# chriskery/slurm-bridge-operator

Measured on AMD Instinct MI355X. Metric: placements/sec + job×node fit evals/sec, 100k nodes×1M jobs, 1–8 MI355X, higher is better.
Workload: dtype int32

## Files before the change

### slurm-bridge-operator_amd/csrc/engine.cpp

```cpp
#include <errno.h>
#include <fcntl.h>
#include <hip/hip_runtime_api.h>
#include <hip/hip_vector_types.h>
#include <rccl/rccl.h>
#include <sys/file.h>
#include <sys/stat.h>
#include <unistd.h>

#include <algorithm>
#include <chrono>
#include <cstdarg>
#include <cstdio>
#include <cstdlib>
#include <cstring>
#include <initializer_list>
#include <map>
#include <mutex>
#include <new>
#include <string>
#include <vector>

#include "../../include/fitgpu.h"
#include "fit_device.h"

using namespace fitgpu;

namespace {

inline int64_t ring_comps(int nc) {
    const int g = std::max(1, std::min(engine_ring_groups(), nc));
    return (nc + g - 1) / g;
}

thread_local std::string g_last_error;

int fail(int code, const char* fmt, ...) {
    char buf[512];
    va_list ap;
    va_start(ap, fmt);
    vsnprintf(buf, sizeof buf, fmt, ap);
    va_end(ap);
    g_last_error = buf;
    return code;
}

#define HIP_TRY(expr)                                                                       \
    do {                                                                                    \
        hipError_t e_ = (expr);                                                             \
        if (e_ != hipSuccess)                                                               \
            return fail(FIT_E_HIP, "%s failed: %s (%s:%d)", #expr, hipGetErrorString(e_),   \
                        __FILE__, __LINE__);                                                \
    } while (0)

#define NCCL_TRY(expr)                                                                      \
    do {                                                                                    \
        ncclResult_t r_ = (expr);                                                           \
        if (r_ != ncclSuccess)                                                              \
            return fail(FIT_E_RCCL, "%s failed: %s", #expr, ncclGetErrorString(r_));        \
    } while (0)

template <class T>
struct DBuf {
    T* p = nullptr;
    size_t cap = 0;
    int ensure(size_t n) {
        if (n <= cap) return 0;
        if (p) (void)hipFree(p);
        p = nullptr;
        cap = 0;
        size_t want = std::max<size_t>(n, 64);
        if (hipMalloc(&p, want * sizeof(T)) != hipSuccess) {
            p = nullptr;
            return fail(FIT_E_OOM, "hipMalloc(%zu bytes) failed", want * sizeof(T));
        }
        cap = want;
        return 0;
    }
    void release() {
        if (p) (void)hipFree(p);
        p = nullptr;
        cap = 0;
    }
    DBuf() = default;
    DBuf(const DBuf&) = delete;
    DBuf& operator=(const DBuf&) = delete;
    ~DBuf() { release(); }
};

template <class T>
struct HBuf {
    T* p = nullptr;
    size_t cap = 0;
    int ensure(size_t n) {
        if (n <= cap) return 0;
        if (p) (void)hipHostFree(p);
        p = nullptr;
        cap = 0;
        size_t want = std::max<size_t>(n, 64);
        if (hipHostMalloc(&p, want * sizeof(T), hipHostMallocDefault) != hipSuccess) {
            p = nullptr;
            return fail(FIT_E_OOM, "hipHostMalloc(%zu bytes) failed", want * sizeof(T));
        }
        cap = want;
        return 0;
    }
    void release() {
        if (p) (void)hipHostFree(p);
        p = nullptr;
        cap = 0;
    }
    HBuf() = default;
    HBuf(const HBuf&) = delete;
    HBuf& operator=(const HBuf&) = delete;
    ~HBuf() { release(); }
};

template <class Row>
struct QueryBufs {
    DBuf<Row> out;
    DBuf<int32_t> bad;
    HBuf<Row> h;
    double ms = -1;
};

int find_root(int* par, int x) {
    while (par[x] != x) x = par[x] = par[par[x]];
    return x;
}

double now_ms() {
    using namespace std::chrono;
    return duration<double, std::milli>(steady_clock::now().time_since_epoch()).count();
}

struct DevArb {
    std::mutex mu;
    int fd = -1;
    std::string path;
};

constexpr const char* FIT_LOCK_DIR_DEFAULT = "/var/run/fitgpu";
int resolve_lock_dir(std::string& dir) {
    const char* e = getenv("FIT_LOCK_DIR");
    if (e && *e) {
        dir = e;
        return 0;
    }
    struct stat sb;
    if (stat(FIT_LOCK_DIR_DEFAULT, &sb) == 0 && S_ISDIR(sb.st_mode)) {
        dir = FIT_LOCK_DIR_DEFAULT;
        return 0;
    }
    dir = "/tmp";
    return 1;
}

DevArb* dev_arb(int device, std::string& err) {
    static std::mutex m;
    static std::map<int, DevArb*> tab;
    std::lock_guard<std::mutex> g(m);
    DevArb*& a = tab[device];
    if (!a) a = new DevArb();
    if (a->fd < 0) {
        char bus[64] = {0};
        if (hipDeviceGetPCIBusId(bus, sizeof bus, device) != hipSuccess) snprintf(bus, sizeof bus, "dev%d", device);
        for (char* q = bus; *q; ++q)
            if (*q == ':' || *q == '/') *q = '_';
        std::string dir;
        (void)resolve_lock_dir(dir);
        a->path = dir + "/fitgpu-" + bus + ".lock";
        a->fd = open(a->path.c_str(), O_RDWR | O_CREAT | O_CLOEXEC, 0666);
        if (a->fd >= 0) (void)fchmod(a->fd, 0666);
        else a->fd = open(a->path.c_str(), O_RDONLY | O_CLOEXEC);
        if (a->fd < 0) {
            err = a->path + ": " + strerror(errno);
            return nullptr;
        }
    }
    return a;
}

struct ArbGuard {
    DevArb* a = nullptr;
    double waited_ms = 0;
    int take(int device) {
        const double t0 = now_ms();
        std::string err;
        DevArb* d = dev_arb(device, err);
        if (!d) return fail(FIT_E_STATE, "device lock %s (set FIT_LOCK_DIR to a writable directory)", err.c_str());
        d->mu.lock();
        int r;
        do r = flock(d->fd, LOCK_EX);
        while (r != 0 && errno == EINTR);
        if (r != 0) {
            d->mu.unlock();
            return fail(FIT_E_STATE, "flock %s: %s", d->path.c_str(), strerror(errno));
        }
        a = d;
        waited_ms = now_ms() - t0;
        return 0;
    }
    ~ArbGuard() {
        if (!a) return;
        (void)flock(a->fd, LOCK_UN);
        a->mu.unlock();
    }
};

}

struct CtxHandles {
    ncclComm_t comm = nullptr;
    hipStream_t st = nullptr;
    hipEvent_t ev[6] = {};
    hipStream_t st2 = nullptr;
    hipEvent_t ev_join = nullptr;
    unsigned* resident = nullptr;
    CtxHandles() = default;
    CtxHandles(const CtxHandles&) = delete;
    CtxHandles& operator=(const CtxHandles&) = delete;
    ~CtxHandles() {
        for (auto& e : ev)
            if (e) (void)hipEventDestroy(e);
        if (ev_join) (void)hipEventDestroy(ev_join);
        if (resident) (void)hipHostFree(resident);
        if (st2) (void)hipStreamDestroy(st2);
        if (st) (void)hipStreamDestroy(st);
        if (comm) (void)ncclCommDestroy(comm);
    }
};

struct fit_ctx : CtxHandles {
    int device = 0;
    int rank = 0, world = 1;
    int shard_mode = FIT_SHARD_AUTO;
    fit_exchange_fn xchg = nullptr;
    void* xchg_user = nullptr;
    HBuf<uint8_t> h_x;
    DBuf<uint64_t> xcount;
    bool force_coll = false;
    bool collective() const { return world > 1 || force_coll; }
    bool persistent = true;
    int32_t small_batch = 2048;
    int32_t small_direct = 128;
    bool small_args = true, sync_spin = true;
    int cls_mode = 3;
    int32_t last_multi = 0;
    bool cls_nodes_ok = false;
    int32_t cls_maxn = 0;
    DBuf<int16_t> jcls;
    DBuf<uint8_t> cls_tab;
    DBuf<int4> cls_dem;
    DBuf<int32_t> cls_n;
    DBuf<unsigned> cls_err;
    HBuf<int32_t> h_cls_n;
    HBuf<unsigned> h_cls_err;
    DBuf<int32_t> small_placed;
    HBuf<int32_t> h_small;
    DBuf<uint8_t> jpack;
    HBuf<uint8_t> h_jpack;
    QueryBufs<fit_why> ex;
    QueryBufs<fit_eta> wh;
    QueryBufs<struct fit_room> rm;
    QueryBufs<fit_eta_k> wk;
    DBuf<int32_t> wk_node, wk_diff;
    HBuf<int32_t> h_wk_node;
    DBuf<unsigned long long> wk_top;
    DBuf<int32_t> ptlk_cnt;
    HBuf<int32_t> h_ptlk;
    DBuf<int32_t> tlr_node, tlr_start, tlr_state, tlr_inv, tlr_cnt, tlr_first, tlr_fill, tlr_touched, tlr_flag, tlr_g;
    DBuf<TlWin> tlr_win;
    DBuf<unsigned long long> tlr_tot;
    HBuf<int32_t> h_tlr_g;
    HBuf<unsigned long long> h_tlr_tot;
    double utl_ms = -1, htl_ms = -1;
    DBuf<int32_t> atl_tc, atl_tm, atl_tg, atl_g;
    HBuf<int32_t> h_atl;
    double atl_ms = -1;
    DBuf<int64_t> free_acc;
    DBuf<fit_free> free_rows;
    double free_ms = -1;
    DBuf<int32_t> vs_off, vs_prio, vs_cpu, vs_mem, vs_gpu, vic_bad, voff;
    HBuf<int32_t> h_vic_bad;
    DBuf<VicEnt> vent;
    bool have_vic = false;
    QueryBufs<fit_evict> pe;
    DBuf<int32_t> pe_prio;
    HBuf<int32_t> h_pe_prio;
    DBuf<uint4> pe_part;
    QueryBufs<fit_evict_k> pk;
    DBuf<int32_t> pk_node, pk_vic;
    HBuf<int32_t> h_pk_pick;
    int cus = 256;
    DBuf<uint8_t> ectl, ering;
    DBuf<CompState> ecs;
    DBuf<CompOut> eco;
    DBuf<int64_t> ebusy;
    HBuf<CompState> h_ecs;
    HBuf<CompOut> h_eco;
    HBuf<int64_t> h_ebusy;
    HBuf<uint32_t> h_err;
    HBuf<TripRec> h_trip;
    DBuf<NodeRec> rec_bak;
    unsigned wd_ticks = 1000000000u;
    HBuf<uint64_t> h_count;
    int wmin = 256, wmax = 8192;

    int32_t n = 0;
    int32_t nn = 0;
    int ncomp = 0;
    int comp_of_part[32];
    std::vector<int32_t> nb;
    DBuf<NodeRec> rec;
    DBuf<int32_t> col_cpu, col_mem, col_gpu, col_av, perm;
    DBuf<uint32_t> col_mask;
    DBuf<int32_t> rb_cpu, rb_mem, rb_gpu;
    std::vector<uint32_t> h_mask;
    std::vector<int32_t> h_perm;
    bool have_nodes = false;
    int64_t loads = 0;

    int32_t np = 0;
    int32_t ptab[128];
    DBuf<int32_t> d_ptab;

    DBuf<int32_t> jcpu, jmem, jgpu, jwall, out, jl, jpk;
    DBuf<uint16_t> jpart, jk;
    DBuf<int8_t> jcomp;
    DBuf<int32_t> jmin;
    DBuf<uint64_t> cand, bnd;
    DBuf<JobRec> wjob;
    DBuf<CompPlan> plan;
    DBuf<CommitResult> res;
    HBuf<CompPlan> h_plan;
    HBuf<CommitResult> h_res;
    DBuf<int32_t> jls;
    HBuf<int32_t> h_jls;

    int32_t tl_slots = 0, tl_slot_min = 0;
    bool have_tl = false;
    DBuf<Seg> slab;
    DBuf<TlHdr> tlhdr;
    DBuf<int32_t> outs, rel_off, rel_slot, rel_cpu, rel_mem, rel_gpu;
    DBuf<uint32_t> tl_err;
    HBuf<uint32_t> h_tl_err;
};

namespace {

int build_ptab(fit_ctx* c) {
    for (int p = 0; p < 32; ++p) c->ptab[96 + p] = c->comp_of_part[p];
    if (c->d_ptab.ensure(128)) return FIT_E_OOM;
    HIP_TRY(hipMemcpyAsync(c->d_ptab.p, c->ptab, sizeof c->ptab, hipMemcpyHostToDevice, c->st));
    return 0;
}

int load_nodes_common(fit_ctx* c, int32_t n) {
    int par[32];
    for (int i = 0; i < 32; ++i) par[i] = i;
    bool used[32] = {false};
    for (int32_t x = 0; x < n; ++x) {
        uint32_t m = c->h_mask[x];
        if (!m) continue;
        int lo = __builtin_ctz(m);
        for (uint32_t r = m; r; r &= r - 1) {
            int b = __builtin_ctz(r);
            used[b] = true;
            int ra = find_root(par, lo), rb = find_root(par, b);
            if (ra != rb) par[std::max(ra, rb)] = std::min(ra, rb);
        }
    }
    int root_comp[32];
    for (int i = 0; i < 32; ++i) root_comp[i] = -1;
    c->ncomp = 0;
    for (int p = 0; p < 32; ++p) {
        c->comp_of_part[p] = -1;
        if (!used[p]) continue;
        int r = find_root(par, p);
        if (root_comp[r] < 0) root_comp[r] = c->ncomp++;
        c->comp_of_part[p] = root_comp[r];
    }
    c->nb.assign(c->ncomp + 1, 0);
    for (int32_t x = 0; x < n; ++x)
        if (c->h_mask[x]) c->nb[c->comp_of_part[__builtin_ctz(c->h_mask[x])] + 1]++;
    for (int k = 0; k < c->ncomp; ++k) {
        if (c->nb[k + 1] > MAX_COMPONENT_NODES)
            return fail(FIT_E_INVAL, "partition component %d has %d nodes (limit %d)", k,
                        c->nb[k + 1], MAX_COMPONENT_NODES);
        c->nb[k + 1] += c->nb[k];
    }
    c->nn = c->nb[c->ncomp];
    {
        int parts_of[32] = {0};
        for (int p = 0; p < 32; ++p)
            if (c->comp_of_part[p] >= 0) ++parts_of[c->comp_of_part[p]];
        c->cls_nodes_ok = c->ncomp > 0 && c->ncomp <= 32;
        c->cls_maxn = 0;
        for (int k = 0; k < c->ncomp; ++k) {
            const int32_t nk = c->nb[k + 1] - c->nb[k];
            c->cls_maxn = std::max(c->cls_maxn, nk);
            if (parts_of[k] != 1) c->cls_nodes_ok = false;
        }
        if (c->cls_maxn > class_max_nodes() || class_lds_bytes(c->cls_maxn) > 160 * 1024)
            c->cls_nodes_ok = false;
    }
    std::vector<int32_t> fill(c->nb.begin(), c->nb.end() - 1), perm(std::max(c->nn, 1));
    for (int32_t x = 0; x < n; ++x)
        if (c->h_mask[x]) perm[fill[c->comp_of_part[__builtin_ctz(c->h_mask[x])]]++] = x;
    if (c->perm.ensure(std::max(c->nn, 1)) || c->rec.ensure(std::max(c->nn, 1))) return FIT_E_OOM;
    HIP_TRY(hipMemcpyAsync(c->perm.p, perm.data(), sizeof(int32_t) * c->nn, hipMemcpyHostToDevice,
                           c->st));
    HIP_TRY(launch_gather_nodes(c->st, c->col_cpu.p, c->col_mem.p, c->col_gpu.p, c->col_av.p,
                                c->col_mask.p, c->perm.p, c->nn, c->rec.p));
    int rc = build_ptab(c);
    if (rc) return rc;
    HIP_TRY(hipStreamSynchronize(c->st));
    perm.resize(c->nn);
    c->h_perm.swap(perm);
    c->n = n;
    c->have_nodes = true;
    c->have_tl = false;
    ++c->loads;
    return 0;
}

int alloc_cols(fit_ctx* c, int32_t n) {
    size_t m = std::max<int32_t>(n, 1);
    if (c->col_cpu.ensure(m) || c->col_mem.ensure(m) || c->col_gpu.ensure(m) ||
        c->col_av.ensure(m) || c->col_mask.ensure(m))
        return FIT_E_OOM;
    return 0;
}

int xchg(fit_ctx* c, int op, void* dbuf, int64_t count) {
    if (!c->collective() || count == 0) return 0;
    if (!c->xchg) {
        switch (op) {
            case FIT_XCHG_ALLGATHER_U64: {
                uint64_t* b = static_cast<uint64_t*>(dbuf);
                NCCL_TRY(ncclAllGather(b + (size_t)c->rank * count, b, count, ncclUint64, c->comm,
                                       c->st));
                return 0;
            }
            case FIT_XCHG_MIN_U64:
                NCCL_TRY(ncclAllReduce(dbuf, dbuf, count, ncclUint64, ncclMin, c->comm, c->st));
                return 0;
            case FIT_XCHG_MAX_I32:
                NCCL_TRY(ncclAllReduce(dbuf, dbuf, count, ncclInt32, ncclMax, c->comm, c->st));
                return 0;
            case FIT_XCHG_MIN_I32:
                NCCL_TRY(ncclAllReduce(dbuf, dbuf, count, ncclInt32, ncclMin, c->comm, c->st));
                return 0;
        }
        return fail(FIT_E_INVAL, "exchange op %d", op);
    }
    const size_t elem = (op == FIT_XCHG_ALLGATHER_U64 || op == FIT_XCHG_MIN_U64) ? 8 : 4;
    const size_t bytes = elem * (size_t)count * (op == FIT_XCHG_ALLGATHER_U64 ? c->world : 1);
    if (c->h_x.ensure(bytes)) return FIT_E_OOM;
    HIP_TRY(hipMemcpyAsync(c->h_x.p, dbuf, bytes, hipMemcpyDeviceToHost, c->st));
    HIP_TRY(hipStreamSynchronize(c->st));
    if (c->xchg(c->xchg_user, op, c->h_x.p, count) != 0)
        return fail(FIT_E_RCCL, "host exchange op %d failed", op);
    HIP_TRY(hipMemcpyAsync(dbuf, c->h_x.p, bytes, hipMemcpyHostToDevice, c->st));
    return 0;
}

const char* trip_site_name(unsigned s) {
    switch (s) {
        case TRIP_WORKER_RING: return "scan worker waiting for a task";
        case TRIP_ROUND_START: return "committer waiting for the round before last";
        case TRIP_HELPER_TILE: return "commit helper waiting for a scan tile";
        case TRIP_HELPER_SNAP: return "commit helper waiting for the decider";
        case TRIP_DECIDER_REC: return "decider waiting for a helper record";
        case TRIP_SINGLE_TILE: return "single-wave commit waiting for a scan tile";
        case TRIP_NO_PROGRESS: return "round resolved no job";
// ... 1326 lines not shown
        c->comp_of_part[p] = -1;
        c->ptab[p] = c->ptab[32 + p] = c->ptab[64 + p] = -1;
        c->ptab[96 + p] = -1;
    }
    int rc = 0;
    if (hipStreamCreateWithFlags(&c->st, hipStreamNonBlocking) != hipSuccess) rc = FIT_E_HIP;
    for (auto& e : c->ev)
        if (!rc && hipEventCreate(&e) != hipSuccess) rc = FIT_E_HIP;
    if (!rc && c->world == 1 && c->force_coll && !c->xchg) {
        ncclUniqueId id;
        ncclResult_t r = ncclGetUniqueId(&id);
        if (r == ncclSuccess) r = ncclCommInitRank(&c->comm, 1, id, 0);
        if (r != ncclSuccess) rc = fail(FIT_E_RCCL, "ncclCommInitRank(1 rank): %s", ncclGetErrorString(r));
    } else if (!rc && c->world > 1 && !c->xchg) {
        if (!o.nccl_id) {
            rc = fail(FIT_E_INVAL, "world > 1 needs nccl_id");
        } else {
            ncclUniqueId id;
            memcpy(&id, o.nccl_id, sizeof id);
            ncclResult_t r = ncclCommInitRank(&c->comm, c->world, id, c->rank);
            if (r != ncclSuccess)
                rc = fail(FIT_E_RCCL, "ncclCommInitRank: %s", ncclGetErrorString(r));
        }
    } else if (rc) {
        fail(rc, "stream/event creation failed");
    }
    if (rc) {
        delete c;
        return rc;
    }
    *out_ctx = c;
    return 0;
}

int fit_set_watchdog_us(fit_ctx* c, int64_t us) {
    if (!c) return fail(FIT_E_INVAL, "null ctx");
    if (us <= 0) {
        c->wd_ticks = 1000000000u;
        if (const char* ev = getenv("FIT_WATCHDOG_MS"))
            c->wd_ticks = (unsigned)std::min<double>(4.29e9, std::max(1.0, atof(ev) * 1e5));
        return 0;
    }
    c->wd_ticks = (unsigned)std::min<int64_t>(us * 100, 4290000000ll);
    return 0;
}

void fit_destroy(fit_ctx* ctx) {
    if (!ctx) return;
    (void)hipSetDevice(ctx->device);
    (void)hipStreamSynchronize(ctx->st);
    delete ctx;
}

static int load_node_cols(fit_ctx* c, int32_t n, const int32_t* cpu, const int32_t* mem, const int32_t* gpu,
                          const int32_t* av, const uint32_t* mask, hipMemcpyKind kind) {
    if (!c) return fail(FIT_E_INVAL, "null ctx");
    if (n < 0 || n > FIT_MAX_NODES || (n > 0 && (!cpu || !mem || !gpu || !av || !mask)))
        return fail(FIT_E_INVAL, "bad node arrays");
    c->have_nodes = c->have_tl = false;
    c->have_vic = false;
    HIP_TRY(hipSetDevice(c->device));
    if (alloc_cols(c, n)) return FIT_E_OOM;
    const size_t b = sizeof(int32_t) * n;
    HIP_TRY(hipMemcpyAsync(c->col_cpu.p, cpu, b, kind, c->st));
    HIP_TRY(hipMemcpyAsync(c->col_mem.p, mem, b, kind, c->st));
    HIP_TRY(hipMemcpyAsync(c->col_gpu.p, gpu, b, kind, c->st));
    HIP_TRY(hipMemcpyAsync(c->col_av.p, av, b, kind, c->st));
    HIP_TRY(hipMemcpyAsync(c->col_mask.p, mask, b, kind, c->st));
    return 0;
}

int fit_load_nodes(fit_ctx* c, int32_t n, const int32_t* cpu, const int32_t* mem,
                   const int32_t* gpu, const int32_t* av, const uint32_t* mask) {
    const int rc = load_node_cols(c, n, cpu, mem, gpu, av, mask, hipMemcpyHostToDevice);
    if (rc) return rc;
    c->h_mask.assign(mask, mask + n);
    return load_nodes_common(c, n);
}

int fit_load_nodes_device(fit_ctx* c, int32_t n, const int32_t* cpu, const int32_t* mem,
                          const int32_t* gpu, const int32_t* av, const uint32_t* mask) {
    const int rc = load_node_cols(c, n, cpu, mem, gpu, av, mask, hipMemcpyDeviceToDevice);
    if (rc) return rc;
    c->h_mask.resize(n);
    HIP_TRY(hipMemcpyAsync(c->h_mask.data(), mask, sizeof(uint32_t) * n, hipMemcpyDeviceToHost, c->st));
    HIP_TRY(hipStreamSynchronize(c->st));
    return load_nodes_common(c, n);
}

int fit_load_partitions(fit_ctx* c, int32_t p, const int32_t* max_time,
                        const int32_t* max_cpus, const int32_t* max_mem) {
    if (!c) return fail(FIT_E_INVAL, "null ctx");
    if (p < 0 || p > FIT_MAX_PARTITIONS || (p > 0 && (!max_time || !max_cpus || !max_mem)))
        return fail(FIT_E_INVAL, "bad partition table (p=%d)", p);
    HIP_TRY(hipSetDevice(c->device));
    c->np = p;
    for (int i = 0; i < 32; ++i) {
        c->ptab[i] = i < p ? max_time[i] : -1;
        c->ptab[32 + i] = i < p ? max_cpus[i] : -1;
        c->ptab[64 + i] = i < p ? max_mem[i] : -1;
    }
    int rc = build_ptab(c);
    if (rc) return rc;
    HIP_TRY(hipStreamSynchronize(c->st));
    return 0;
}

static int check_place_args(fit_ctx* c, int32_t j, std::initializer_list<const void*> arrays, int32_t kmax) {
    const int rc = check_job_args(c, j, arrays, nullptr, 0);
    if (rc) return rc;
    if (kmax < 1 || kmax > FIT_MAX_K)
        return fail(FIT_E_INVAL, "kmax=%d outside [1, %d]", kmax, FIT_MAX_K);
    return 0;
}

constexpr int32_t kPackJobs = 16384;

int fit_place(fit_ctx* c, int32_t j, const int32_t* cpu, const int32_t* mem, const int32_t* gpu,
              const int32_t* wall, const uint16_t* part, const uint16_t* nk, int32_t kmax,
              int32_t* out, fit_stats* stats) {
    int rc = check_place_args(c, j, {cpu, mem, gpu, wall, part, out}, kmax);
    if (rc) return rc;
    HIP_TRY(hipSetDevice(c->device));
    size_t m = std::max(j, 1);
    if (c->out.ensure(m * kmax + 2 + FIT_MAX_PARTITIONS + 1)) return FIT_E_OOM;
    if (c->small_args && j <= SMALL_ARGJ && j <= c->small_direct && !c->collective()) {
        SmallBatch hb;
        memcpy(hb.cpu, cpu, sizeof(int32_t) * j);
        memcpy(hb.mem, mem, sizeof(int32_t) * j);
        memcpy(hb.gpu, gpu, sizeof(int32_t) * j);
        memcpy(hb.wall, wall, sizeof(int32_t) * j);
        memcpy(hb.part, part, sizeof(uint16_t) * j);
        if (nk) memcpy(hb.nk, nk, sizeof(uint16_t) * j);
        bool done = false;
        rc = place_impl(c, j, nullptr, nullptr, nullptr, nullptr, nullptr, nk, kmax, c->out.p, stats, out, &done,
                        &hb);
        if (rc) return rc;
        if (!done) return fail(FIT_E_HIP, "direct placement did not return its placements");
        return 0;
    }
// ... 673 lines not shown
```

### slurm-bridge-operator_amd/csrc/fit_device.h

```cpp
#pragma once
#include <hip/hip_runtime_api.h>
#include <hip/hip_vector_types.h>
#include <stdint.h>

namespace fitgpu {

#ifndef FIT_KS
#define FIT_KS 16
#endif
constexpr int KS = FIT_KS;
static_assert(KS >= 2 && KS <= 16 && (KS & (KS - 1)) == 0, "FIT_KS must be a power of two in [2, 16]");
constexpr int SCAN_WAVES = 8;
constexpr int SCAN_JOBS = 64;
#ifndef FIT_MIN_SUB
#define FIT_MIN_SUB 64
#endif
constexpr int MIN_SUB = FIT_MIN_SUB;
#ifndef FIT_MAX_SLICES
#define FIT_MAX_SLICES (128 / FIT_KS)
#endif
constexpr int MAX_SLICES = FIT_MAX_SLICES;
#ifndef FIT_TL_KS
#define FIT_TL_KS 4
#endif
// ... 280 lines not shown
                            const ExplainComps& C, const int32_t* jcpu, const int32_t* jmem, const int32_t* jgpu,
                            const int32_t* jwall, const uint16_t* jpart, const int32_t* jprio, int32_t kmax,
                            int32_t nj, const int8_t* jcomp, const int32_t* jl, const int32_t* live, int slices,
                            void* part, void* out, int32_t* out_node, int32_t* out_vic);

enum TripSite : unsigned {
    TRIP_NONE = 0,
    TRIP_WORKER_RING = 1,
    TRIP_ROUND_START = 2,
    TRIP_HELPER_TILE = 3,
    TRIP_HELPER_SNAP = 4,
    TRIP_DECIDER_REC = 5,
    TRIP_SINGLE_TILE = 6,
    TRIP_NO_PROGRESS = 7,
    TRIP_NO_KERNEL = 8,
    TRIP_PEER = 9,
};
struct TripRec {
    unsigned claim, site, comp, round;
    unsigned arg, q_head, q_tail, pubt;
    unsigned tdone, need, block, pad;
    unsigned long long waited;
    unsigned long long when;
};


hipError_t launch_scan(int blocks, hipStream_t st, const NodeRec* rec, const int32_t* jl,
                       const int32_t* jcpu, const int32_t* jmem, const int32_t* jgpu,
                       const int32_t* jwall, const uint16_t* jpart, const uint16_t* jk,
                       const CompPlan* plan, int ncomp, uint64_t* cand, uint64_t* bnd,
                       JobRec* wjob);
hipError_t launch_commit(int ncomp, int epl, size_t lds_bytes, hipStream_t st, NodeRec* rec,
                         const CompPlan* plan, const uint64_t* cand, int64_t rank_stride,
                         int nranks, const uint64_t* bnd, const JobRec* wjob, int32_t* out,
                         int kmax, CommitResult* res);
hipError_t launch_prefilter(hipStream_t st, const int32_t* jcpu, const int32_t* jmem,
                            const int32_t* jgpu, const int32_t* jwall, const uint16_t* jpart, const uint16_t* jk,
                            int32_t nj, int32_t kmax, const int32_t* ptab, int32_t np,
                            int32_t* out, int8_t* jcomp, int32_t* jmin = nullptr);
size_t joblists_scratch_ints(int32_t nj);
hipError_t launch_joblists(hipStream_t st, const int8_t* jcomp, int32_t nj, int ncomp,
                           int32_t* scratch, int32_t* g, int32_t* jb, int32_t* mb, int32_t* jl,
                           int32_t* jpk);
hipError_t launch_small_args(hipStream_t st, int ncomp, NodeRec* rec, const SmallComps& C, const int32_t* ptab,
                             int32_t np, const SmallBatch& B, bool has_nk, int32_t nj, int32_t kmax, int32_t* out,
                             int32_t* stat);
hipError_t launch_small(hipStream_t st, int ncomp, NodeRec* rec, const SmallComps& C,
                        const int32_t* ptab, int32_t np, const int32_t* jcpu, const int32_t* jmem,
                        const int32_t* jgpu, const int32_t* jwall, const uint16_t* jpart,
                        const uint16_t* jk, int32_t nj, int32_t kmax, int32_t* out, int32_t* stat);
hipError_t launch_gather_nodes(hipStream_t st, const int32_t* cpu, const int32_t* mem,
                               const int32_t* gpu, const int32_t* av, const uint32_t* mask,
                               const int32_t* perm, int32_t nn, NodeRec* rec);
hipError_t launch_scatter_nodes(hipStream_t st, const NodeRec* rec, int32_t nn, int32_t* cpu,
                                int32_t* mem, int32_t* gpu);
size_t engine_lds_bytes(int32_t max_component_nodes);
size_t class_lds_bytes(int32_t max_component_nodes);
int class_max();
int class_table_slots();
size_t class_slot_bytes();
int class_max_nodes();
hipError_t launch_classify(hipStream_t st, const int8_t* jcomp, const int32_t* jcpu, const int32_t* jmem,
                           const int32_t* jgpu, const uint16_t* jpart, int32_t nj, void* tab, int4* dem,
                           int32_t* ncls, int16_t* jcls);
hipError_t launch_class(hipStream_t st, int ncomp, size_t lds, NodeRec* rec, const int32_t* nbv, uint32_t owned,
                        const int32_t* jb, const int32_t* jl, const int32_t* jwall, const uint16_t* jk,
                        const int16_t* jcls, const int4* dem, const int32_t* ncls, int32_t kmax, int32_t* out,
                        CompOut* co, unsigned* err);
hipError_t launch_class_out(hipStream_t st, int32_t* out, int64_t n, const NodeRec* rec);
size_t engine_ctl_bytes();
size_t engine_ctl_error_offset();
size_t engine_ctl_trip_offset();
size_t engine_ring_bytes();
size_t engine_ring_tasks();
int engine_ring_groups();
int engine_blocks_per_cu(size_t lds);
hipError_t launch_engine(int blocks, size_t lds, hipStream_t st, void* ctl, void* ring,
                         const void* cs, void* co, CompPlan* plans, int ncomp, NodeRec* rec,
                         const int32_t* jl, const int32_t* jcpu, const int32_t* jmem,
                         const int32_t* jgpu, const int32_t* jwall, const uint16_t* jpart,
                         const uint16_t* jk, uint64_t* cand, uint64_t* bnd, JobRec* wjob,
                         int32_t* out, int kmax, int64_t* wbusy, const int32_t* jpk, unsigned wd,
                         const int32_t* jmin, const EngineCompIds& ids);
hipError_t launch_build_tl(hipStream_t st, const int32_t* cpu, const int32_t* mem,
                           const int32_t* gpu, const int32_t* av, const uint32_t* mask,
                           const int32_t* perm, int32_t nn, int32_t H, int32_t slot_min,
                           const int32_t* off, const int32_t* rs, const int32_t* rc,
                           const int32_t* rm, const int32_t* rg, Seg* slab, TlHdr* hdr,
                           uint32_t* err);
hipError_t launch_scan_tl(int blocks, hipStream_t st, const Seg* slab, const TlHdr* hdr,
                          const int32_t* jl, const int32_t* jcpu, const int32_t* jmem,
                          const int32_t* jgpu, const int32_t* jwall, const uint16_t* jpart,
                          const CompPlan* plan, int ncomp, uint64_t* cand, uint64_t* bnd,
                          JobRec* wjob, int32_t H, int32_t slot_min);
size_t commit_tl_lds_bytes(int32_t max_component_nodes);
int commit_tl_runs(int32_t max_component_nodes);
hipError_t launch_commit_tl(int ncomp, int epl, size_t lds, hipStream_t st, Seg* slab,
                            TlHdr* hdr, const CompPlan* plan, const uint64_t* cand,
                            int64_t rank_stride, int nranks, const uint64_t* bnd,
                            const JobRec* wjob, const int32_t* perm, int32_t* out, int32_t* outs,
                            CommitResult* res, int32_t H, int32_t R);
int engine_tl_runs(int32_t max_component_nodes);
size_t engine_tl_lds_bytes(int32_t max_component_nodes);
int engine_tl_blocks_per_cu(size_t lds, int mode);
size_t engine_tl_scan_lds_bytes();
hipError_t launch_engine_tl(int blocks, size_t lds, hipStream_t st, void* ctl, void* ring,
// ... 13 lines not shown
```

### slurm-bridge-operator_amd/csrc/fit_kernels.hip

```cpp
#include "fit_common.h"

namespace fitgpu {

__global__ __launch_bounds__(SCAN_WAVES * 64) void k_scan(
    const NodeRec* __restrict__ rec, const int32_t* __restrict__ jl,
    const int32_t* __restrict__ jcpu, const int32_t* __restrict__ jmem,
    const int32_t* __restrict__ jgpu, const int32_t* __restrict__ jwall,
    const uint16_t* __restrict__ jpart, const uint16_t* __restrict__ jk,
    const CompPlan* __restrict__ plan, int ncomp, uint64_t* __restrict__ cand,
    uint64_t* __restrict__ bnd, JobRec* __restrict__ wjob) {
    __shared__ uint64_t xk[SCAN_WAVES / 2][KS][64];
    const int c = find_comp(plan, ncomp, blockIdx.x);
    const CompPlan P = plan[c];
    const int local = blockIdx.x - P.blk0;
    const int tile = __builtin_amdgcn_readfirstlane(local / P.nslice);
    const int s = __builtin_amdgcn_readfirstlane(local - tile * P.nslice);
    scan_tile<false, KS>(P, tile, s, rec, jl, jcpu, jmem, jgpu, jwall, jpart, jk, cand, bnd, wjob, xk);
}

template <int EPL>
__global__ __launch_bounds__(64) void k_commit(
    NodeRec* __restrict__ rec, const CompPlan* __restrict__ plan,
    const uint64_t* __restrict__ cand, int64_t rank_stride, int nranks,
    const uint64_t* __restrict__ bnd, const JobRec* __restrict__ wjob,
// ... 34 lines not shown
    const int32_t* __restrict__ jcpu, const int32_t* __restrict__ jmem,
    const int32_t* __restrict__ jgpu, const int32_t* __restrict__ jwall, const uint16_t* __restrict__ jpart,
    const uint16_t* __restrict__ jk, int32_t nj, int32_t kmax,
    const int32_t* __restrict__ ptab ,
    int32_t np, int32_t* __restrict__ out, int8_t* __restrict__ jcomp, int32_t* __restrict__ jmin) {
    __shared__ int32_t smin[MIN ? 3 * ENGINE_MAXC : 1];
    if constexpr (MIN) {
        if (threadIdx.x < 3 * ENGINE_MAXC) smin[threadIdx.x] = INT32_MAX;
        __syncthreads();
    }
    const int q = blockIdx.x * blockDim.x + threadIdx.x;
    if (q < nj) {
        bool rej;
        int k;
        const int code = job_code(q, jcpu, jmem, jgpu, jwall, jpart, jk, kmax, ptab, np, &rej, &k);
        jcomp[q] = (int8_t)code;
        for (int i = 0; i < kmax; ++i) out[(int64_t)q * kmax + i] = (rej && i < k) ? -2 : -1;
        if constexpr (MIN) {
            if (code >= 0) {
                const int cc = code & 0x3f;
                atomicMin(&smin[3 * cc], jcpu[q]);
                atomicMin(&smin[3 * cc + 1], jmem[q]);
                atomicMin(&smin[3 * cc + 2], jgpu ? jgpu[q] : 0);
            }
        }
    }
    if constexpr (MIN) {
        __syncthreads();
        if (threadIdx.x < 3 * ENGINE_MAXC) {
            const int32_t v = smin[threadIdx.x];
            if (v != INT32_MAX &&
                v < __hip_atomic_load(&jmin[threadIdx.x], __ATOMIC_RELAXED, __HIP_MEMORY_SCOPE_AGENT))
                atomicMin(&jmin[threadIdx.x], v);
        }
    }
}

__global__ void k_gather_nodes(const int32_t* __restrict__ cpu, const int32_t* __restrict__ mem,
                               const int32_t* __restrict__ gpu, const int32_t* __restrict__ av,
                               const uint32_t* __restrict__ mask, const int32_t* __restrict__ perm,
                               int32_t nn, NodeRec* __restrict__ rec) {
    const int i = blockIdx.x * blockDim.x + threadIdx.x;
    if (i >= nn) return;
    const int x = perm[i];
    NodeRec r;
    r.cpu = max(cpu[x], -1);
    r.mem = max(mem[x], -1);
    r.gpu = max(gpu[x], -1);
    r.avail = max(av[x], -1);
    r.mask = mask[x];
    r.orig = x;
    r.pad0 = r.pad1 = 0;
    rec[i] = r;
}

__global__ void k_scatter_nodes(const NodeRec* __restrict__ rec, int32_t nn,
                                int32_t* __restrict__ cpu, int32_t* __restrict__ mem,
                                int32_t* __restrict__ gpu) {
    const int i = blockIdx.x * blockDim.x + threadIdx.x;
    if (i >= nn) return;
    const NodeRec r = rec[i];
    if (r.cpu >= 0) cpu[r.orig] = r.cpu;
    if (r.mem >= 0) mem[r.orig] = r.mem;
    if (r.gpu >= 0) gpu[r.orig] = r.gpu;
}


constexpr int JL_BLOCK = 1024;
constexpr int JL_MAXC = ENGINE_MAXC;

__global__ __launch_bounds__(JL_BLOCK) void k_jl_count(const int8_t* __restrict__ jcomp, int32_t nj,
                                                       int ncomp, int32_t* __restrict__ bc,
                                                       int32_t* __restrict__ bm,
                                                       int32_t* __restrict__ g) {
    __shared__ int32_t wc[JL_BLOCK / 64][JL_MAXC], wm[JL_BLOCK / 64][JL_MAXC];
    const int q = blockIdx.x * JL_BLOCK + threadIdx.x;
    const int wave = threadIdx.x >> 6, lane = threadIdx.x & 63;
    const int k = q < nj ? jcomp[q] : -1;
    const int comp = k >= 0 ? (k & 0x3f) : -1;
    const bool multi = k >= 0 && (k & 0x40);
    for (int cc = 0; cc < ncomp; ++cc) {
        const uint64_t m = __ballot(comp == cc), mm = __ballot(comp == cc && multi);
        if (lane == 0) {
            wc[wave][cc] = __popcll(m);
            wm[wave][cc] = __popcll(mm);
        }
    }
    __shared__ int32_t brj, bbad;
    if (threadIdx.x == 0) brj = bbad = 0;
    __syncthreads();
    const uint64_t rj = __ballot(k == -2), bad = __ballot(k == -3);
    if (lane == 0 && rj) atomicAdd(&brj, (int)__popcll(rj));
    if (lane == 0 && bad) bbad = 1;
    __syncthreads();
    if (threadIdx.x == 0 && brj) atomicAdd(&g[0], brj);
    if (threadIdx.x == 0 && bbad) atomicOr(&g[1], 1);
    if ((int)threadIdx.x < ncomp) {
        int a = 0, b = 0;
        for (int w = 0; w < JL_BLOCK / 64; ++w) {
            a += wc[w][threadIdx.x];
            b += wm[w][threadIdx.x];
        }
        bc[blockIdx.x * JL_MAXC + threadIdx.x] = a;
        bm[blockIdx.x * JL_MAXC + threadIdx.x] = b;
    }
}
// ... 390 lines not shown
extern "C" int fit_debug_commit_stamps(unsigned long long* out ) {
    return hipMemcpyFromSymbol(out, HIP_SYMBOL(g_stamps), sizeof(g_stamps)) == hipSuccess ? 0 : -2;
}
#endif

hipError_t launch_prefilter(hipStream_t st, const int32_t* jcpu, const int32_t* jmem,
                            const int32_t* jgpu, const int32_t* jwall, const uint16_t* jpart, const uint16_t* jk,
                            int32_t nj, int32_t kmax, const int32_t* ptab, int32_t np,
                            int32_t* out, int8_t* jcomp, int32_t* jmin) {
    if (nj == 0) return hipSuccess;
    if (jmin)
        hipLaunchKernelGGL(k_prefilter<true>, dim3((nj + 255) / 256), dim3(256), 0, st, jcpu, jmem, jgpu,
                           jwall, jpart, jk, nj, kmax, ptab, np, out, jcomp, jmin);
    else
        hipLaunchKernelGGL(k_prefilter<false>, dim3((nj + 255) / 256), dim3(256), 0, st, jcpu, jmem, jgpu,
                           jwall, jpart, jk, nj, kmax, ptab, np, out, jcomp, jmin);
    return hipGetLastError();
}

size_t joblists_scratch_ints(int32_t nj) { return (size_t)2 * ((nj + JL_BLOCK - 1) / JL_BLOCK) * JL_MAXC; }

hipError_t launch_joblists(hipStream_t st, const int8_t* jcomp, int32_t nj, int ncomp,
                           int32_t* scratch, int32_t* g, int32_t* jb, int32_t* mb, int32_t* jl,
                           int32_t* jpk) {
    if (ncomp > JL_MAXC) return hipErrorInvalidValue;
    const int nblocks = (nj + JL_BLOCK - 1) / JL_BLOCK;
    int32_t* bc = scratch;
    int32_t* bm = scratch + (size_t)nblocks * JL_MAXC;
    hipError_t e = hipMemsetAsync(g, 0, 2 * sizeof(int32_t), st);
    if (e != hipSuccess) return e;
    if (nj > 0) {
        hipLaunchKernelGGL(k_jl_count, dim3(nblocks), dim3(JL_BLOCK), 0, st, jcomp, nj, ncomp, bc, bm, g);
    }
    hipLaunchKernelGGL(k_jl_scan, dim3(1), dim3(1024), 0, st, nblocks, ncomp, bc, bm, jb, mb);
    if (nj > 0) {
        hipLaunchKernelGGL(k_jl_scatter, dim3(nblocks), dim3(JL_BLOCK), 0, st, jcomp, nj, ncomp, bc,
                           bm, jb, mb, jl, jpk);
    } else {
        e = hipMemsetAsync(jpk, 0, sizeof(int32_t), st);
        if (e != hipSuccess) return e;
    }
    return hipGetLastError();
}

hipError_t launch_gather_nodes(hipStream_t st, const int32_t* cpu, const int32_t* mem,
                               const int32_t* gpu, const int32_t* av, const uint32_t* mask,
                               const int32_t* perm, int32_t nn, NodeRec* rec) {
    if (nn == 0) return hipSuccess;
    hipLaunchKernelGGL(k_gather_nodes, dim3((nn + 255) / 256), dim3(256), 0, st, cpu, mem, gpu,
                       av, mask, perm, nn, rec);
    return hipGetLastError();
}

hipError_t launch_scatter_nodes(hipStream_t st, const NodeRec* rec, int32_t nn, int32_t* cpu,
                                int32_t* mem, int32_t* gpu) {
    if (nn == 0) return hipSuccess;
    hipLaunchKernelGGL(k_scatter_nodes, dim3((nn + 255) / 256), dim3(256), 0, st, rec, nn, cpu,
                       mem, gpu);
    return hipGetLastError();
}

}
```

Baseline: 38.87 million.

## Cache node partition layout across loads and detect unchanged masks on device

```diff
diff --git a/slurm-bridge-operator_amd/csrc/engine.cpp b/slurm-bridge-operator_amd/csrc/engine.cpp
--- a/slurm-bridge-operator_amd/csrc/engine.cpp
+++ b/slurm-bridge-operator_amd/csrc/engine.cpp
@@ -22,6 +22,7 @@
 
 #include "../../include/fitgpu.h"
 #include "fit_device.h"
+#include "fit_layout.h"
 
 using namespace fitgpu;
 
@@ -122,11 +123,6 @@
     HBuf<Row> h;
     double ms = -1;
 };
-
-int find_root(int* par, int x) {
-    while (par[x] != x) x = par[x] = par[par[x]];
-    return x;
-}
 
 double now_ms() {
     using namespace std::chrono;
@@ -230,7 +226,7 @@
     }
 };
 
-struct fit_ctx : CtxHandles {
+struct fit_ctx : CtxHandles, NodeLayout {
     int device = 0;
     int rank = 0, world = 1;
     int shard_mode = FIT_SHARD_AUTO;
@@ -247,7 +243,6 @@
     int cls_mode = 3;
     int32_t last_multi = 0;
     bool cls_nodes_ok = false;
-    int32_t cls_maxn = 0;
     DBuf<int16_t> jcls;
     DBuf<uint8_t> cls_tab;
     DBuf<int4> cls_dem;
@@ -306,17 +301,16 @@
     HBuf<uint64_t> h_count;
     int wmin = 256, wmax = 8192;
 
-    int32_t n = 0;
-    int32_t nn = 0;
-    int ncomp = 0;
-    int comp_of_part[32];
-    std::vector<int32_t> nb;
     DBuf<NodeRec> rec;
     DBuf<int32_t> col_cpu, col_mem, col_gpu, col_av, perm;
     DBuf<uint32_t> col_mask;
     DBuf<int32_t> rb_cpu, rb_mem, rb_gpu;
-    std::vector<uint32_t> h_mask;
-    std::vector<int32_t> h_perm;
+    DBuf<unsigned long long> lay_diff;
+    HBuf<unsigned long long> h_lay_diff;
+    unsigned long long lay_stamp = 0;
+    std::vector<uint32_t> mask_in;
+    HBuf<uint32_t> pin_mask;
+    HBuf<int32_t> pin_perm;
     bool have_nodes = false;
     int64_t loads = 0;
 
@@ -355,72 +349,41 @@
     return 0;
 }
 
-int load_nodes_common(fit_ctx* c, int32_t n) {
-    int par[32];
-    for (int i = 0; i < 32; ++i) par[i] = i;
-    bool used[32] = {false};
-    for (int32_t x = 0; x < n; ++x) {
-        uint32_t m = c->h_mask[x];
-        if (!m) continue;
-        int lo = __builtin_ctz(m);
-        for (uint32_t r = m; r; r &= r - 1) {
-            int b = __builtin_ctz(r);
-            used[b] = true;
-            int ra = find_root(par, lo), rb = find_root(par, b);
-            if (ra != rb) par[std::max(ra, rb)] = std::min(ra, rb);
-        }
-    }
-    int root_comp[32];
-    for (int i = 0; i < 32; ++i) root_comp[i] = -1;
-    c->ncomp = 0;
-    for (int p = 0; p < 32; ++p) {
-        c->comp_of_part[p] = -1;
-        if (!used[p]) continue;
-        int r = find_root(par, p);
-        if (root_comp[r] < 0) root_comp[r] = c->ncomp++;
-        c->comp_of_part[p] = root_comp[r];
-    }
-    c->nb.assign(c->ncomp + 1, 0);
-    for (int32_t x = 0; x < n; ++x)
-        if (c->h_mask[x]) c->nb[c->comp_of_part[__builtin_ctz(c->h_mask[x])] + 1]++;
-    for (int k = 0; k < c->ncomp; ++k) {
-        if (c->nb[k + 1] > MAX_COMPONENT_NODES)
-            return fail(FIT_E_INVAL, "partition component %d has %d nodes (limit %d)", k,
-                        c->nb[k + 1], MAX_COMPONENT_NODES);
-        c->nb[k + 1] += c->nb[k];
-    }
-    c->nn = c->nb[c->ncomp];
-    {
-        int parts_of[32] = {0};
-        for (int p = 0; p < 32; ++p)
-            if (c->comp_of_part[p] >= 0) ++parts_of[c->comp_of_part[p]];
-        c->cls_nodes_ok = c->ncomp > 0 && c->ncomp <= 32;
-        c->cls_maxn = 0;
-        for (int k = 0; k < c->ncomp; ++k) {
-            const int32_t nk = c->nb[k + 1] - c->nb[k];
-            c->cls_maxn = std::max(c->cls_maxn, nk);
-            if (parts_of[k] != 1) c->cls_nodes_ok = false;
-        }
-        if (c->cls_maxn > class_max_nodes() || class_lds_bytes(c->cls_maxn) > 160 * 1024)
-            c->cls_nodes_ok = false;
-    }
-    std::vector<int32_t> fill(c->nb.begin(), c->nb.end() - 1), perm(std::max(c->nn, 1));
-    for (int32_t x = 0; x < n; ++x)
-        if (c->h_mask[x]) perm[fill[c->comp_of_part[__builtin_ctz(c->h_mask[x])]]++] = x;
-    if (c->perm.ensure(std::max(c->nn, 1)) || c->rec.ensure(std::max(c->nn, 1))) return FIT_E_OOM;
-    HIP_TRY(hipMemcpyAsync(c->perm.p, perm.data(), sizeof(int32_t) * c->nn, hipMemcpyHostToDevice,
-                           c->st));
+int layout_cache_mode() {
+    static const int mode = getenv("FIT_LAYOUT_CACHE") ? atoi(getenv("FIT_LAYOUT_CACHE")) : 1;
+    return mode;
+}
+
+int rebuild_layout(fit_ctx* c, int32_t n) {
+    int32_t bad_nodes = 0;
+    const int bad = layout_build(*c, n, MAX_COMPONENT_NODES, &bad_nodes);
+    if (bad >= 0)
+        return fail(FIT_E_INVAL, "partition component %d has %d nodes (limit %d)", bad, bad_nodes,
+                    MAX_COMPONENT_NODES);
+    c->cls_nodes_ok = c->cls_shape_ok && c->cls_maxn <= class_max_nodes() &&
+                      class_lds_bytes(c->cls_maxn) <= 160 * 1024;
+    if (c->perm.ensure(std::max(c->nn, 1)) || c->rec.ensure(std::max(c->nn, 1)) ||
+        c->pin_perm.ensure(std::max(c->nn, 1)))
+        return FIT_E_OOM;
+    if (c->nn) {
+        memcpy(c->pin_perm.p, c->h_perm.data(), sizeof(int32_t) * c->nn);
+        HIP_TRY(hipMemcpyAsync(c->perm.p, c->pin_perm.p, sizeof(int32_t) * c->nn, hipMemcpyHostToDevice, c->st));
+    }
+    return build_ptab(c);
+}
+
+int gather_nodes(fit_ctx* c) {
     HIP_TRY(launch_gather_nodes(c->st, c->col_cpu.p, c->col_mem.p, c->col_gpu.p, c->col_av.p,
                                 c->col_mask.p, c->perm.p, c->nn, c->rec.p));
-    int rc = build_ptab(c);
-    if (rc) return rc;
-    HIP_TRY(hipStreamSynchronize(c->st));
-    perm.resize(c->nn);
-    c->h_perm.swap(perm);
+    return 0;
+}
+
+int nodes_loaded(fit_ctx* c, int32_t n) {
     c->n = n;
     c->have_nodes = true;
     c->have_tl = false;
     ++c->loads;
+    c->layout_valid = true;
     return 0;
 }
 
@@ -1853,15 +1816,27 @@
     delete ctx;
 }
 
-static int load_node_cols(fit_ctx* c, int32_t n, const int32_t* cpu, const int32_t* mem, const int32_t* gpu,
-                          const int32_t* av, const uint32_t* mask, hipMemcpyKind kind) {
+static int check_node_args(fit_ctx* c, int32_t n, const int32_t* cpu, const int32_t* mem, const int32_t* gpu,
+                           const int32_t* av, const uint32_t* mask) {
     if (!c) return fail(FIT_E_INVAL, "null ctx");
     if (n < 0 || n > FIT_MAX_NODES || (n > 0 && (!cpu || !mem || !gpu || !av || !mask)))
         return fail(FIT_E_INVAL, "bad node arrays");
+    return 0;
+}
+
+static int load_node_cols(fit_ctx* c, int32_t n, const int32_t* cpu, const int32_t* mem, const int32_t* gpu,
+                          const int32_t* av, const uint32_t* mask, hipMemcpyKind kind, bool test_mask) {
     c->have_nodes = c->have_tl = false;
     c->have_vic = false;
     HIP_TRY(hipSetDevice(c->device));
     if (alloc_cols(c, n)) return FIT_E_OOM;
+    if (test_mask) {
+        if (!c->lay_diff.p) {
+            if (c->lay_diff.ensure(1) || c->h_lay_diff.ensure(1)) return FIT_E_OOM;
+            HIP_TRY(hipMemsetAsync(c->lay_diff.p, 0, sizeof(unsigned long long), c->st));
+        }
+        HIP_TRY(launch_mask_differs(c->st, c->col_mask.p, mask, n, ++c->lay_stamp, c->lay_diff.p));
+    }
     const size_t b = sizeof(int32_t) * n;
     HIP_TRY(hipMemcpyAsync(c->col_cpu.p, cpu, b, kind, c->st));
     HIP_TRY(hipMemcpyAsync(c->col_mem.p, mem, b, kind, c->st));
@@ -1873,20 +1848,63 @@
 
 int fit_load_nodes(fit_ctx* c, int32_t n, const int32_t* cpu, const int32_t* mem,
                    const int32_t* gpu, const int32_t* av, const uint32_t* mask) {
-    const int rc = load_node_cols(c, n, cpu, mem, gpu, av, mask, hipMemcpyHostToDevice);
-    if (rc) return rc;
-    c->h_mask.assign(mask, mask + n);
-    return load_nodes_common(c, n);
+    int rc = check_node_args(c, n, cpu, mem, gpu, av, mask);
+    if (rc) return rc;
+    const bool hit = layout_cache_mode() != 0 && layout_hit(*c, n, mask);
+    c->layout_valid = false;
+    rc = load_node_cols(c, n, cpu, mem, gpu, av, mask, hipMemcpyHostToDevice, false);
+    if (rc) return rc;
+    if (!hit) {
+        c->h_mask.assign(mask, mask + n);
+        rc = rebuild_layout(c, n);
+        if (rc) return rc;
+    }
+    rc = gather_nodes(c);
+    if (rc) return rc;
+    HIP_TRY(hipStreamSynchronize(c->st));
+    return nodes_loaded(c, n);
 }
 
 int fit_load_nodes_device(fit_ctx* c, int32_t n, const int32_t* cpu, const int32_t* mem,
                           const int32_t* gpu, const int32_t* av, const uint32_t* mask) {
-    const int rc = load_node_cols(c, n, cpu, mem, gpu, av, mask, hipMemcpyDeviceToDevice);
-    if (rc) return rc;
-    c->h_mask.resize(n);
-    HIP_TRY(hipMemcpyAsync(c->h_mask.data(), mask, sizeof(uint32_t) * n, hipMemcpyDeviceToHost, c->st));
+    int rc = check_node_args(c, n, cpu, mem, gpu, av, mask);
+    if (rc) return rc;
+    const int mode = layout_cache_mode();
+    const bool cand = mode != 0 && layout_same_shape(*c, n);
+    c->layout_valid = false;
+    const bool on_dev = cand && n > 0 && mode != 2;
+    rc = load_node_cols(c, n, cpu, mem, gpu, av, mask, hipMemcpyDeviceToDevice, on_dev);
+    if (rc) return rc;
+    bool hit = cand && n == 0;
+    if (on_dev) {
+        rc = gather_nodes(c);
+        if (rc) return rc;
+        HIP_TRY(hipMemcpyAsync(c->h_lay_diff.p, c->lay_diff.p, sizeof(unsigned long long), hipMemcpyDeviceToHost,
+                               c->st));
+        HIP_TRY(hipStreamSynchronize(c->st));
+        hit = *c->h_lay_diff.p != c->lay_stamp;
+        if (hit) return nodes_loaded(c, n);
+    }
+    if (!hit) {
+        const bool on_host = cand && !on_dev;
+        std::vector<uint32_t>& to = on_host ? c->mask_in : c->h_mask;
+        if (c->pin_mask.ensure(std::max(n, 1))) return FIT_E_OOM;
+        HIP_TRY(hipMemcpyAsync(c->pin_mask.p, mask, sizeof(uint32_t) * n, hipMemcpyDeviceToHost, c->st));
+        HIP_TRY(hipStreamSynchronize(c->st));
+        to.assign(c->pin_mask.p, c->pin_mask.p + n);
+        if (on_host) {
+            hit = layout_same_words(*c, n, c->mask_in.data());
+            if (!hit) c->h_mask.swap(c->mask_in);
+        }
+    }
+    if (!hit) {
+        rc = rebuild_layout(c, n);
+        if (rc) return rc;
+    }
+    rc = gather_nodes(c);
+    if (rc) return rc;
     HIP_TRY(hipStreamSynchronize(c->st));
-    return load_nodes_common(c, n);
+    return nodes_loaded(c, n);
 }
 
 int fit_load_partitions(fit_ctx* c, int32_t p, const int32_t* max_time,
diff --git a/slurm-bridge-operator_amd/csrc/fit_device.h b/slurm-bridge-operator_amd/csrc/fit_device.h
--- a/slurm-bridge-operator_amd/csrc/fit_device.h
+++ b/slurm-bridge-operator_amd/csrc/fit_device.h
@@ -356,6 +356,8 @@
 hipError_t launch_gather_nodes(hipStream_t st, const int32_t* cpu, const int32_t* mem,
                                const int32_t* gpu, const int32_t* av, const uint32_t* mask,
                                const int32_t* perm, int32_t nn, NodeRec* rec);
+hipError_t launch_mask_differs(hipStream_t st, const uint32_t* loaded, const uint32_t* mask, int32_t n,
+                               unsigned long long stamp, unsigned long long* diff);
 hipError_t launch_scatter_nodes(hipStream_t st, const NodeRec* rec, int32_t nn, int32_t* cpu,
                                 int32_t* mem, int32_t* gpu);
 size_t engine_lds_bytes(int32_t max_component_nodes);
diff --git a/slurm-bridge-operator_amd/csrc/fit_kernels.hip b/slurm-bridge-operator_amd/csrc/fit_kernels.hip
--- a/slurm-bridge-operator_amd/csrc/fit_kernels.hip
+++ b/slurm-bridge-operator_amd/csrc/fit_kernels.hip
@@ -110,6 +110,12 @@
     r.orig = x;
     r.pad0 = r.pad1 = 0;
     rec[i] = r;
+}
+
+__global__ void k_mask_differs(const uint32_t* __restrict__ loaded, const uint32_t* __restrict__ mask,
+                               int32_t n, unsigned long long stamp, unsigned long long* __restrict__ diff) {
+    const int i = blockIdx.x * blockDim.x + threadIdx.x;
+    if (i < n && loaded[i] != mask[i]) *diff = stamp;
 }
 
 __global__ void k_scatter_nodes(const NodeRec* __restrict__ rec, int32_t nn,
@@ -606,6 +612,13 @@
     return hipGetLastError();
 }
 
+hipError_t launch_mask_differs(hipStream_t st, const uint32_t* loaded, const uint32_t* mask, int32_t n,
+                               unsigned long long stamp, unsigned long long* diff) {
+    if (n == 0) return hipSuccess;
+    hipLaunchKernelGGL(k_mask_differs, dim3((n + 255) / 256), dim3(256), 0, st, loaded, mask, n, stamp, diff);
+    return hipGetLastError();
+}
+
 hipError_t launch_scatter_nodes(hipStream_t st, const NodeRec* rec, int32_t nn, int32_t* cpu,
                                 int32_t* mem, int32_t* gpu) {
     if (nn == 0) return hipSuccess;
diff --git a/slurm-bridge-operator_amd/csrc/fit_layout.h b/slurm-bridge-operator_amd/csrc/fit_layout.h
--- /dev/null
+++ b/slurm-bridge-operator_amd/csrc/fit_layout.h
@@ -0,0 +1,93 @@
+#pragma once
+#include <algorithm>
+#include <cstdint>
+#include <cstring>
+#include <vector>
+
+namespace fitgpu {
+
+struct NodeLayout {
+    bool layout_valid = false;
+    int32_t n = 0;
+    int32_t nn = 0;
+    int ncomp = 0;
+    int comp_of_part[32] = {};
+    std::vector<int32_t> nb;
+    std::vector<uint32_t> h_mask;
+    std::vector<int32_t> h_perm;
+    bool cls_shape_ok = false;
+    int32_t cls_maxn = 0;
+    std::vector<int32_t> lay_fill;
+};
+
+inline bool layout_same_shape(const NodeLayout& L, int32_t n) {
+    return L.layout_valid && n >= 0 && n == L.n && L.h_mask.size() == (size_t)n;
+}
+inline bool layout_same_words(const NodeLayout& L, int32_t n, const uint32_t* mask) {
+    if (n == 0) return true;
+    return mask && memcmp(mask, L.h_mask.data(), sizeof(uint32_t) * (size_t)n) == 0;
+}
+inline bool layout_hit(const NodeLayout& L, int32_t n, const uint32_t* mask) {
+    return layout_same_shape(L, n) && layout_same_words(L, n, mask);
+}
+
+inline int layout_build(NodeLayout& L, int32_t n, int32_t max_comp_nodes, int32_t* bad_nodes) {
+    const uint32_t* mask = L.h_mask.data();
+    int par[32];
+    for (int i = 0; i < 32; ++i) par[i] = i;
+    auto find_root = [&par](int x) {
+        while (par[x] != x) x = par[x] = par[par[x]];
+        return x;
+    };
+    bool used[32] = {false};
+    for (int32_t x = 0; x < n; ++x) {
+        uint32_t m = mask[x];
+        if (!m) continue;
+        int lo = __builtin_ctz(m);
+        for (uint32_t r = m; r; r &= r - 1) {
+            int b = __builtin_ctz(r);
+            used[b] = true;
+            int ra = find_root(lo), rb = find_root(b);
+            if (ra != rb) par[std::max(ra, rb)] = std::min(ra, rb);
+        }
+    }
+    int root_comp[32];
+    for (int i = 0; i < 32; ++i) root_comp[i] = -1;
+    L.ncomp = 0;
+    for (int p = 0; p < 32; ++p) {
+        L.comp_of_part[p] = -1;
+        if (!used[p]) continue;
+        int r = find_root(p);
+        if (root_comp[r] < 0) root_comp[r] = L.ncomp++;
+        L.comp_of_part[p] = root_comp[r];
+    }
+    L.nb.assign(L.ncomp + 1, 0);
+    for (int32_t x = 0; x < n; ++x)
+        if (mask[x]) L.nb[L.comp_of_part[__builtin_ctz(mask[x])] + 1]++;
+    for (int k = 0; k < L.ncomp; ++k) {
+        if (L.nb[k + 1] > max_comp_nodes) {
+            *bad_nodes = L.nb[k + 1];
+            return k;
+        }
+        L.nb[k + 1] += L.nb[k];
+    }
+    L.nn = L.nb[L.ncomp];
+    {
+        int parts_of[32] = {0};
+        for (int p = 0; p < 32; ++p)
+            if (L.comp_of_part[p] >= 0) ++parts_of[L.comp_of_part[p]];
+        L.cls_shape_ok = L.ncomp > 0 && L.ncomp <= 32;
+        L.cls_maxn = 0;
+        for (int k = 0; k < L.ncomp; ++k) {
+            L.cls_maxn = std::max(L.cls_maxn, L.nb[k + 1] - L.nb[k]);
+            if (parts_of[k] != 1) L.cls_shape_ok = false;
+        }
+    }
+    L.lay_fill.assign(L.nb.begin(), L.nb.end() - 1);
+    L.h_perm.resize(L.nn);
+    for (int32_t x = 0; x < n; ++x)
+        if (mask[x]) L.h_perm[L.lay_fill[L.comp_of_part[__builtin_ctz(mask[x])]]++] = x;
+    return -1;
+}
+
+}
```

Result: no change. 39.12 million (median of 6 runs) (+0.6%).
